# Cc19245/gaussian-splatting_CC-Comments

Hardware: AMD Instinct MI355X
Metric: train iters/sec (fwd+bwd rasterize) @1980x1080, 1M Gaussians (higher is better)
Workload: dtype f32; 1 GPU; C3: 1000000 Gaussians, SH deg 3, 1980x1080, mu=-5.0, seed 0; P=1000000, parallelism=single view

## Files before the change

__graft_entry__.py:

```python
import os
import subprocess
import sys

ROOT = os.path.dirname(os.path.abspath(__file__))
PKG = os.path.join(ROOT, "gaussian-splatting_cc-comments_amd")
CSRC = os.path.join(PKG, "csrc")
LIB = os.path.join(PKG, "libgsr_hip.so")
for p in (ROOT, PKG):
    if p not in sys.path:
        sys.path.insert(0, p)


def _stale(target, sources):
    if not os.path.exists(target):
        return True
    t = os.path.getmtime(target)
    return any(os.path.getmtime(s) > t for s in sources)


def build(force=False):
    srcs = [os.path.join(CSRC, f) for f in os.listdir(CSRC) if f.endswith((".hip", ".h", ".inc"))] + \
           [os.path.join(ROOT, "include", h) for h in ("gsr.h", "gsr_aux.h", "gsr_aa.h", "gsr_cam.h", "gsr_absgrad.h", "gsr_contrib.h", "gsr_features.h", "gsr_distortion.h", "gsr_median.h", "gsr_normals.h", "gsr_camera_model.h", "gsr_cam_cm.h")] + [os.path.join(CSRC, "Makefile")]
    if force or _stale(LIB, srcs):
        jobs = str(min(8, os.cpu_count() or 1))
        subprocess.check_call(["make", "-C", CSRC, "-j", jobs] + (["-B"] if force else []))
    subprocess.check_call(["make", "-C", os.path.join(ROOT, "tests", "cpp")], stdout=subprocess.DEVNULL)
    from oracle import oracle as _oracle
    _oracle.build(force=force)
    import diff_gaussian_rasterization
    from diff_gaussian_rasterization import _C
    _C.lib()


def smoke():
    import numpy as np
    import torch

    import gsr_scene
    from diff_gaussian_rasterization import GaussianRasterizationSettings, GaussianRasterizer
    from oracle import oracle

    assert torch.cuda.is_available(), "smoke() needs a GPU"
    dev = torch.device("cuda:0")
    scene = gsr_scene.make_scene(2000, -3.0, sh_degree=3, seed=3)
    cam = gsr_scene.make_camera(200, 120)
    to = lambda t: t.to(dev)
    means = to(scene.means3D).requires_grad_(True)
    shs = to(scene.shs).requires_grad_(True)
    opac = to(scene.opacities).requires_grad_(True)
    scales = to(scene.scales).requires_grad_(True)
    rots = to(scene.rotations).requires_grad_(True)
    means2D = torch.zeros_like(means, requires_grad=True)
    settings = GaussianRasterizationSettings(
        image_height=cam.image_height, image_width=cam.image_width, tanfovx=cam.tanfovx, tanfovy=cam.tanfovy,
        bg=to(scene.bg), scale_modifier=1.0, viewmatrix=to(cam.world_view_transform),
# ... 29 lines not shown
```

gaussian-splatting_cc-comments_amd/csrc/api.hip:

```cpp
#include <stdarg.h>
#include <stdio.h>
#include <string.h>

#include <atomic>
#include <cmath>
#include <mutex>
#include <string>
#include <vector>

#include "gsr_internal.h"
#include "../../include/gsr_aa.h"
#include "../../include/gsr_contrib.h"
#include "../../include/gsr_features.h"
#include "../../include/gsr_distortion.h"
#include "../../include/gsr_median.h"
#include "../../include/gsr_normals.h"

#define GSR_MAX_DEVICES 64
#ifndef GSR_COLOR_BESIDE_WGS
#define GSR_COLOR_BESIDE_WGS 2
#endif
#define GSR_COLOR_BESIDE_MAX_P 1500000

static thread_local char g_err[512] = "";

int gsr_fail(int code, const char* fmt, ...)
{
	va_list ap;
	va_start(ap, fmt);
	vsnprintf(g_err, sizeof g_err, fmt, ap);
	va_end(ap);
	return code;
}

int gsr_check_hip(hipError_t e, const char* what)
{
	if (e == hipSuccess) return GSR_OK;
	return gsr_fail(GSR_ERR_HIP, "%s: %s", what, hipGetErrorString(e));
}

int gsr_stage_done(hipStream_t s, int debug, const char* stage)
{
	hipError_t e = hipGetLastError();
	if (e != hipSuccess) return gsr_fail(GSR_ERR_HIP, "launch of %s failed: %s", stage, hipGetErrorString(e));
	if (debug & GSR_DEBUG_SYNC) {
		e = hipStreamSynchronize(s);
		if (e != hipSuccess) return gsr_fail(GSR_ERR_HIP, "[HIP ERROR] in stage %s: %s", stage, hipGetErrorString(e));
	}
	return GSR_OK;
}

extern "C" const char* gsr_last_error(void) { return g_err; }
extern "C" const char* gsr_version(void) { return "gsr-hip gfx950 r4"; }

struct ProfEntry { const char* name; hipEvent_t a, b; };
struct ProfRecorder {
	hipStream_t stream;
	bool on = false, open = false;
	std::vector<ProfEntry> ev;
	size_t used = 0;
	char only[64] = "";
};
static std::mutex g_prof_mu;
static std::vector<ProfRecorder*> g_prof;
static std::atomic<int> g_prof_active{0};

static ProfRecorder* prof_find(hipStream_t s, bool create)
{
	for (ProfRecorder* r : g_prof)
		if (r->stream == s) return r;
	if (!create) return nullptr;
	ProfRecorder* r = new ProfRecorder();
	r->stream = s;
	g_prof.push_back(r);
	return r;
}

static ProfEntry& prof_next(ProfRecorder* r, const char* name)
{
	if (r->used == r->ev.size()) {
		ProfEntry e;
		e.name = name;
		(void)hipEventCreate(&e.a);
		(void)hipEventCreate(&e.b);
		r->ev.push_back(e);
	}
// ... 266 lines not shown
{
	gsr_binning_layout l;
	gsr_binning_layout_of(P, R, W, H, &l);
	char* b = (char*)blob;
	GsrBinning bn;
	bn.point_list = (uint32_t*)(b + l.point_list);
	bn.point_list_alt = (uint32_t*)(b + l.point_list_alt);
	bn.tile_keys = (uint32_t*)(b + l.tile_keys);
	bn.tile_keys_alt = (uint32_t*)(b + l.tile_keys_alt);
	bn.sort_table = (void*)(b + l.sort_table);
	bn.checkpoints = (float4*)(b + l.checkpoints);
	return bn;
}

extern "C" uint32_t gsr_get_higher_msb(uint32_t n)
{
	uint32_t msb = sizeof(n) * 4;
	uint32_t step = msb;
	while (step > 1) {
		step /= 2;
		if (n >> msb) msb += step; else msb -= step;
	}
	if (n >> msb) msb++;
	return msb;
}

struct GsrThreadDevice {
	hipStream_t aux_stream = nullptr;
	hipEvent_t aux_fork = nullptr, aux_join = nullptr;
	uint32_t* status_host = nullptr;
	hipEvent_t status_event = nullptr;
	hipStream_t copy_stream = nullptr;
	hipEvent_t copy_fork = nullptr;
};
struct GsrThreadState { GsrThreadDevice dev[GSR_MAX_DEVICES]; };
static thread_local GsrThreadState g_thread;

extern "C" int gsr_thread_release(void)
{
	g_err[0] = 0;
	int rc = GSR_OK;
	for (int d = 0; d < GSR_MAX_DEVICES; d++) {
		GsrThreadDevice& t = g_thread.dev[d];
		if (t.aux_stream) { (void)hipStreamSynchronize(t.aux_stream); if (hipStreamDestroy(t.aux_stream) != hipSuccess) rc = GSR_ERR_HIP; }
		if (t.aux_fork && hipEventDestroy(t.aux_fork) != hipSuccess) rc = GSR_ERR_HIP;
		if (t.aux_join && hipEventDestroy(t.aux_join) != hipSuccess) rc = GSR_ERR_HIP;
		if (t.status_event && hipEventDestroy(t.status_event) != hipSuccess) rc = GSR_ERR_HIP;
		if (t.copy_stream) { (void)hipStreamSynchronize(t.copy_stream); if (hipStreamDestroy(t.copy_stream) != hipSuccess) rc = GSR_ERR_HIP; }
		if (t.copy_fork && hipEventDestroy(t.copy_fork) != hipSuccess) rc = GSR_ERR_HIP;
		if (t.status_host && hipHostFree(t.status_host) != hipSuccess) rc = GSR_ERR_HIP;
		t = GsrThreadDevice();
	}
	if (rc) { (void)hipGetLastError(); return gsr_fail(rc, "gsr_thread_release: a HIP resource could not be freed"); }
	return GSR_OK;
}

static bool gsr_helper_stream(hipStream_t* stream, hipEvent_t* e0, hipEvent_t* e1)
{
	if (*stream) return true;
	hipStream_t st = nullptr;
	hipEvent_t a = nullptr, b = nullptr;
	if (hipStreamCreateWithFlags(&st, hipStreamNonBlocking) == hipSuccess && hipEventCreateWithFlags(&a, hipEventDisableTiming) == hipSuccess &&
	    (!e1 || hipEventCreateWithFlags(&b, hipEventDisableTiming) == hipSuccess)) {
		*stream = st; *e0 = a;
		if (e1) *e1 = b;
		return true;
// ... 40 lines not shown
{
	g_err[0] = 0;
	hipStream_t s = (hipStream_t)stream;
	GsrPreprocessArgs a = in;
	const int P = a.P, width = a.W, height = a.H;
	if (!num_rendered_host) return gsr_fail(GSR_ERR_INVALID_ARGUMENT, "num_rendered_host is NULL");
	*num_rendered_host = 0;
	if (P < 0 || width <= 0 || height <= 0) return gsr_fail(GSR_ERR_INVALID_ARGUMENT, "bad P / image size");
	if (P == 0) return GSR_OK;
	if (!a.means3D || !a.opacities || !a.viewmatrix || (!a.projmatrix && !cm) || !geometry)
		return gsr_fail(GSR_ERR_INVALID_ARGUMENT, "gsr_forward_preprocess: required pointer is NULL");
	if (!a.colors_precomp && !a.shs)
		return gsr_fail(GSR_ERR_INVALID_ARGUMENT, "For non-RGB, provide precomputed Gaussian colors!");
	if (!a.colors_precomp && (a.M <= 0 || (a.D + 1) * (a.D + 1) > a.M || a.D < 0 || a.D > 3 || !a.cam_pos))
		return gsr_fail(GSR_ERR_INVALID_ARGUMENT, "SH degree %d needs %d coefficients, M = %d", a.D, (a.D + 1) * (a.D + 1), a.M);
	if (!a.cov3D_precomp && (!a.scales || !a.rotations))
		return gsr_fail(GSR_ERR_INVALID_ARGUMENT, "provide scales+rotations or cov3D_precomp");
	if (width > 65535 * GSR_TILE_X || height > 65535 * GSR_TILE_Y)
		return gsr_fail(GSR_ERR_INVALID_ARGUMENT, "image too large for 16-bit tile coordinates");
	if (!aligned16(geometry)) return gsr_fail(GSR_ERR_INVALID_ARGUMENT, "geometry buffer must be 16-byte aligned");

	if (a.leaf && (a.M > 1 && !a.shs_rest)) return gsr_fail(GSR_ERR_INVALID_ARGUMENT, "leaf mode: features_rest is NULL");
	if (a.leaf && a.M > 16) return gsr_fail(GSR_ERR_INVALID_ARGUMENT, "leaf mode: at most 16 SH coefficients (degree 3), M = %d", a.M);
	a.focal_y = height / (2.0f * a.tan_fovy);
	a.focal_x = width / (2.0f * a.tan_fovx);
	if (cm) { a.focal_x = cm->fx; a.focal_y = cm->fy; }
	a.g = gsr_geometry_view(geometry, P);

	int rc;
	int device = 0;
	if ((rc = gsr_check_hip(hipGetDevice(&device), "hipGetDevice"))) return rc;
	if (device < 0 || device >= GSR_MAX_DEVICES) return gsr_fail(GSR_ERR_INVALID_ARGUMENT, "device index %d not supported", device);
	GsrThreadDevice& td = g_thread.dev[device];
	const bool col_pairs = gsr_tilebin_applies(width, height) && !(debug & GSR_DEBUG_TILE_SORT);
	a.trim = (col_pairs && !(debug & GSR_DEBUG_NO_TRIM)) ? 1 : 0;
	const bool color = gsr_preprocess_needs_color(a);
#ifdef GSR_AB_FORCE_RADIX_DEPTH
	const bool bucket = false;
#else
	const bool bucket = gsr_bucket_sort_applies(P) && !(debug & GSR_DEBUG_RADIX_DEPTH);
#endif
	const bool beside = color && !(debug & (GSR_DEBUG_SYNC | GSR_DEBUG_SERIAL)) && !gsr_prof_records_all(s) &&
	                    gsr_helper_stream(&td.aux_stream, &td.aux_fork, &td.aux_join);
	GsrJoinOnExit join(s);
	gsr_launch_zero_status(a.g.status, s, beside ? td.aux_fork : nullptr);
	if (beside) {
		if ((rc = gsr_check_hip(hipStreamWaitEvent(td.aux_stream, td.aux_fork, 0), "hipStreamWaitEvent(fork)"))) return rc;
		gsr_launch_preprocess_color(a, td.aux_stream, P <= GSR_COLOR_BESIDE_MAX_P ? GSR_COLOR_BESIDE_WGS : 0, aux);
		if (hipEventRecord(td.aux_join, td.aux_stream) != hipSuccess) {
			(void)hipStreamSynchronize(td.aux_stream);
			return gsr_fail(GSR_ERR_HIP, "hipEventRecord(join) failed");
		}
		join.arm(td.aux_join);
	}
	const bool copy_beside = !(debug & (GSR_DEBUG_SYNC | GSR_DEBUG_SERIAL)) && !gsr_prof_records_all(s) &&
	                         gsr_helper_stream(&td.copy_stream, &td.copy_fork, nullptr);
	{
		GsrProfScope p(s, "preprocess");
		gsr_launch_preprocess(a, s, copy_beside ? td.copy_fork : nullptr, aux, aa, cm);
	}
	if ((rc = gsr_stage_done(s, debug, "preprocess"))) return rc;
	if (color && !beside) {
		GsrProfScope p(s, "preprocess_color");
		gsr_launch_preprocess_color(a, s, 0, aux);
	}
	if ((rc = gsr_stage_done(s, debug, "preprocess_color"))) return rc;

	if (!td.status_host) {
		if ((rc = gsr_check_hip(hipHostMalloc((void**)&td.status_host, GSR_STATUS_WORDS * 4, hipHostMallocDefault), "hipHostMalloc"))) return rc;
	}
	if (!td.status_event) {
		if ((rc = gsr_check_hip(hipEventCreateWithFlags(&td.status_event, hipEventDisableTiming), "hipEventCreate"))) return rc;
	}
	uint32_t* status_host = td.status_host;
	hipEvent_t ev = td.status_event;
	if (copy_beside && (rc = gsr_check_hip(hipStreamWaitEvent(td.copy_stream, td.copy_fork, 0), "hipStreamWaitEvent(copy fork)"))) return rc;
	hipStream_t cs = copy_beside ? td.copy_stream : s;
	GsrDrainOnExit drain;
	if (copy_beside) drain.arm(td.copy_stream);
	if ((rc = gsr_check_hip(hipMemcpyAsync(status_host, a.g.status, GSR_STATUS_WORDS * 4, hipMemcpyDeviceToHost, cs), "hipMemcpyAsync(num_rendered)"))) return rc;
	if ((rc = gsr_check_hip(hipEventRecord(ev, cs), "hipEventRecord"))) return rc;
	const uint32_t* bias = a.g.status + GSR_STATUS_NEGMIN;
	{
		GsrProfScope p(s, "depth_sort");
		if (bucket) {
			gsr_launch_depth_bucket_sort(a.g, P, col_pairs ? gsr_tilebin_seg(a.g, P) : nullptr, s);
			if (col_pairs) gsr_launch_tilebin_col_hist(a.g, P, 0, s, true);
			else gsr_launch_sorted_block_sums(a.g, P, 0, s);
		} else {
			gsr_radix_sort_passes(a.g.depth_keys, a.g.perm, a.g.depth_keys_alt, a.g.perm_alt, (size_t)P, 32, 4, 0, 3, a.g.sort_table, bias, 4, s);
			if (col_pairs) gsr_launch_tilebin_col_hist(a.g, P, 1, s);
			else gsr_launch_sorted_block_sums(a.g, P, 1, s);
			gsr_launch_slot_base_finish(a.g.slot_base, a.g.block_tiles, a.g.status, (size_t)P, s);
		}
	}
	if ((rc = gsr_stage_done(s, debug, "depth_sort"))) return rc;
	if ((rc = gsr_check_hip(hipEventSynchronize(ev), "hipEventSynchronize(num_rendered)"))) return rc;
// ... 981 lines not shown
```

gaussian-splatting_cc-comments_amd/csrc/gsr_internal.h:

```cpp
#pragma once
#include <hip/hip_runtime.h>
#include <hip/hip_ext.h>
#include <stddef.h>
#include <stdint.h>

#include <type_traits>

#include "../../include/gsr.h"
#include "../../include/gsr_aux.h"
#include "../../include/gsr_cam.h"
#include "../../include/gsr_absgrad.h"
#include "../../include/gsr_camera_model.h"
#include "../../include/gsr_cam_cm.h"
#include "gsr_device.h"

#define GSR_PREPROCESS_BLOCK 256
#define GSR_COUNT_PARTS 64
#define GSR_STATUS_NEGMIN (4 + GSR_COUNT_PARTS)
#define GSR_STATUS_MAX (4 + 2 * GSR_COUNT_PARTS)
#define GSR_STATUS_WORDS (4 + 3 * GSR_COUNT_PARTS)

#ifndef GSR_SLOT_COOP
#define GSR_SLOT_COOP 30
#endif
// ... 95 lines not shown
		if (aux == GSR_AUX_INVDEPTH) with_leaf(std::integral_constant<int, GSR_AUX_INVDEPTH>{}, AA);
		else if (aux) with_leaf(std::integral_constant<int, GSR_AUX_DEPTH>{}, AA);
		else with_leaf(std::integral_constant<int, 0>{}, AA);
	};
	if (aa) with_aux(std::true_type{});
	else with_aux(std::false_type{});
}

struct GsrPreprocessArgs {
	int P, D, M, W, H;
	const float* means3D;
	const float* shs;
	const float* colors_precomp;
	const float* opacities;
	const float* scales;
	float scale_modifier;
	const float* rotations;
	const float* cov3D_precomp;
	const float* viewmatrix;
	const float* projmatrix;
	const float* cam_pos;
	float tan_fovx, tan_fovy, focal_x, focal_y;
	int prefiltered;
	int trim;
	int* radii;
	GsrGeometry g;
	int leaf;
	const float* shs_rest;
};

void gsr_launch_preprocess(const GsrPreprocessArgs& a, hipStream_t s, hipEvent_t done, int aux, int aa, const gsr_camera_model* cm = nullptr);
void gsr_launch_zero_status(uint32_t* status, hipStream_t s, hipEvent_t done);
bool gsr_preprocess_needs_color(const GsrPreprocessArgs& a);
void gsr_launch_preprocess_color(const GsrPreprocessArgs& a, hipStream_t s, int wgs_per_cu, int aux);
void gsr_launch_mark_visible(int P, const float* means3D, const float* viewmatrix, uint8_t* present, hipStream_t s);

void gsr_launch_sorted_block_sums(GsrGeometry g, int P, int result_in_alt, hipStream_t s);
void gsr_launch_duplicate_keys(GsrGeometry g, int P, int W, void* keys, int key_bytes, uint32_t* vals, uint32_t* clear, size_t clear_words, hipStream_t s);
void gsr_launch_tile_ranges(const void* tile_keys, int key_bytes, int64_t R, uint2* ranges, int ntiles, uint32_t* valid, hipStream_t s);
void gsr_launch_tile_order(GsrImage img, int ntiles, bool backward, int64_t num_rendered, bool split, hipStream_t s, bool normalise_empty = false);
uint32_t gsr_tile_order_max_split(int ntiles);
uint32_t gsr_tile_order_max_segments(int ntiles);

bool gsr_tilebin_applies(int W, int H);
size_t gsr_tilebin_col_clear_words(size_t P);
size_t gsr_tilebin_col_table_bytes(size_t P);
size_t gsr_tilebin_row_clear_words(size_t R);
size_t gsr_tilebin_row_table_bytes(size_t R);
void gsr_launch_tilebin_col_hist(GsrGeometry g, int P, int result_in_alt, hipStream_t s, bool seg_ready = false);
uint4* gsr_tilebin_seg(GsrGeometry g, int P);
uint4* gsr_tilebin_recs(GsrGeometry g, int P);
void gsr_launch_tilebin_col_scatter(GsrGeometry g, int P, GsrBinning b, int64_t R, hipStream_t s);
void gsr_launch_tilebin_row_hist(GsrGeometry g, int P, GsrBinning b, int64_t R, hipStream_t s);
void gsr_launch_tilebin_row_scatter(GsrGeometry g, int P, GsrBinning b, int64_t R, uint2* ranges, int W, int H, hipStream_t s);

int gsr_radix_num_passes(int nbits_total);
size_t gsr_radix_table_bytes(size_t n);
size_t gsr_radix_clear_words(size_t n);
void gsr_launch_slot_base_finish(uint32_t* slot_base, const uint32_t* block_tiles, uint32_t* status, size_t n, hipStream_t s);
void gsr_radix_sort_passes(void* k0, uint32_t* v0, void* k1, uint32_t* v1, size_t n, int nbits_total, int npass_total,
                           int pass_first, int pass_count, void* table_mem, const uint32_t* bias, int key_bytes, hipStream_t s);
void gsr_radix_sort_u32(void* k0, uint32_t* v0, void* k1, uint32_t* v1, size_t n, int nbits_total, void* table_mem,
                        int* result_in_first, int clear_table, int key_bytes, hipStream_t s);
void gsr_radix_top_pass(const uint32_t* k0, uint32_t* k1, const uint2* rec_in, uint4* rec_out, size_t n, void* table_mem, const uint32_t* bias, hipStream_t s,
                        uint32_t* slot_base, const uint32_t* block_tiles, uint32_t* status);
int gsr_radix_top_chunks(size_t n);
#ifndef GSR_BUCKET_SORT_MAX_P
// ... 110 lines not shown
```

gaussian-splatting_cc-comments_amd/csrc/preprocess.hip:

```cpp
#include "gsr_internal.h"
#include "gsr_rect_trim.h"
#include "gsr_aa.h"
#include "gsr_camera_model.h"

__device__ __forceinline__ float gsr_sh_channel(int deg, const float* sh, int ch, float x, float y, float z)
{
#define SH(k) sh[(k) * 3 + ch]
	float result = GSR_SH_C0 * SH(0);
	if (deg > 0) {
		result = result - GSR_SH_C1 * y * SH(1) + GSR_SH_C1 * z * SH(2) - GSR_SH_C1 * x * SH(3);
		if (deg > 1) {
			float xx = x * x, yy = y * y, zz = z * z;
			float xy = x * y, yz = y * z, xz = x * z;
			result = result + GSR_SH_C2[0] * xy * SH(4) + GSR_SH_C2[1] * yz * SH(5) +
			         GSR_SH_C2[2] * (2.0f * zz - xx - yy) * SH(6) + GSR_SH_C2[3] * xz * SH(7) +
			         GSR_SH_C2[4] * (xx - yy) * SH(8);
			if (deg > 2) {
				result = result + GSR_SH_C3[0] * y * (3.0f * xx - yy) * SH(9) + GSR_SH_C3[1] * xy * z * SH(10) +
				         GSR_SH_C3[2] * y * (4.0f * zz - xx - yy) * SH(11) +
				         GSR_SH_C3[3] * z * (2.0f * zz - 3.0f * xx - 3.0f * yy) * SH(12) +
				         GSR_SH_C3[4] * x * (4.0f * zz - xx - yy) * SH(13) + GSR_SH_C3[5] * z * (xx - yy) * SH(14) +
				         GSR_SH_C3[6] * x * (xx - 3.0f * yy) * SH(15);
			}
		}
	}
#undef SH
	return result + 0.5f;
}

template <bool LEAF, int AUX, bool AA, bool CM>
__global__ void __launch_bounds__(GSR_PREPROCESS_BLOCK) gsr_preprocess_kernel(
	typename std::conditional<CM, GsrWithCameraModel<GsrPreprocessArgs>, GsrPreprocessArgs>::type a, uint32_t* __restrict__ clear, size_t clear_words,
	uint32_t* __restrict__ clear2, size_t clear2_words)
{
	const int idx = blockIdx.x * GSR_PREPROCESS_BLOCK + threadIdx.x;
	GsrVec3 p_orig = {0.f, 0.f, 0.f};
// ... 104 lines not shown
	for (int off = 32; off > 0; off >>= 1) {
		kneg = max(kneg, (uint32_t)__shfl_xor(kneg, off, 64));
		kmax = max(kmax, (uint32_t)__shfl_xor(kmax, off, 64));
	}
	if ((threadIdx.x & 63) == 63) { wsum[threadIdx.x >> 6] = incl; wneg[threadIdx.x >> 6] = kneg; wmax[threadIdx.x >> 6] = kmax; }
	__syncthreads();
	{
		uint32_t before = 0, t = 0;
#pragma unroll
		for (int w = 0; w < GSR_PREPROCESS_BLOCK / 64; w++) {
			if (w < (int)(threadIdx.x >> 6)) before += wsum[w];
			t += wsum[w];
		}
		if (idx < a.P) a.g.slot_base[idx] = before + incl - tiles;
		if (threadIdx.x == 0) {
			a.g.block_tiles[blockIdx.x] = t;
			uint32_t n2 = 0, m2 = 0;
#pragma unroll
			for (int w = 0; w < GSR_PREPROCESS_BLOCK / 64; w++) { n2 = max(n2, wneg[w]); m2 = max(m2, wmax[w]); }
			if (t) {
				const int part = blockIdx.x & (GSR_COUNT_PARTS - 1);
				atomicAdd(&a.g.status[4 + part], t);
				atomicMax(&a.g.status[GSR_STATUS_NEGMIN + part], n2);
				atomicMax(&a.g.status[GSR_STATUS_MAX + part], m2);
			}
		}
	}
	for (size_t w = (size_t)blockIdx.x * GSR_PREPROCESS_BLOCK + threadIdx.x; w < clear_words; w += (size_t)gridDim.x * GSR_PREPROCESS_BLOCK)
		clear[w] = 0u;
	for (size_t w = (size_t)blockIdx.x * GSR_PREPROCESS_BLOCK + threadIdx.x; w < clear2_words; w += (size_t)gridDim.x * GSR_PREPROCESS_BLOCK)
		clear2[w] = 0u;
}

template <bool LEAF, int AUX>
__global__ void __launch_bounds__(GSR_PREPROCESS_BLOCK) gsr_preprocess_color_kernel(GsrPreprocessArgs a, int sh_via_lds)
{
	__shared__ float4 s_sh[GSR_PREPROCESS_BLOCK / 64][32 * GSR_SH_ROW4];
	const int idx = blockIdx.x * GSR_PREPROCESS_BLOCK + threadIdx.x;
	GsrVec3 p_orig = {0.f, 0.f, 0.f};
	if (idx < a.P) { p_orig.x = a.means3D[3 * idx]; p_orig.y = a.means3D[3 * idx + 1]; p_orig.z = a.means3D[3 * idx + 2]; }
	float row[48];
	if (sh_via_lds) {
		const int lane = threadIdx.x & 63, wave = threadIdx.x >> 6;
		const int wave_first = blockIdx.x * GSR_PREPROCESS_BLOCK + wave * 64;
		const int nrows = min(64, a.P - wave_first);
		if (LEAF) {
			GsrShLinFetch v;
			gsr_sh_lin_fetch(v, a.shs, a.shs_rest, wave_first, max(nrows, 0), lane);
			float* lin = reinterpret_cast<float*>(s_sh[wave]);
#pragma unroll
			for (int half = 0; half < 2; half++) {
				gsr_sh_lin_commit_half(lin, v, lane, half);
				__builtin_amdgcn_wave_barrier();
				if ((lane >> 5) == half) gsr_sh_linh_row_get(lin, lane & 31, row);
				__builtin_amdgcn_wave_barrier();
			}
		} else {
			float4 v[12];
			gsr_sh_rows_fetch(v, a.shs, wave_first, max(nrows, 0), lane);
#pragma unroll
			for (int half = 0; half < 2; half++) {
				gsr_sh_rows_commit_half(s_sh[wave], v, nrows, lane, half);
				__builtin_amdgcn_wave_barrier();
				if ((lane >> 5) == half) gsr_sh_row_get(s_sh[wave], lane & 31, row);
				__builtin_amdgcn_wave_barrier();
			}
		}
	}
	if (idx >= a.P) return;
	if (gsr_transform_point_4x3(p_orig, a.viewmatrix).z <= 0.2f) return;

	float dx = p_orig.x - a.cam_pos[0], dy = p_orig.y - a.cam_pos[1], dz = p_orig.z - a.cam_pos[2];
	float len = sqrtf(dx * dx + dy * dy + dz * dz);
	dx = dx / len; dy = dy / len; dz = dz / len;
	const float* sh = a.shs + (size_t)idx * a.M * 3;
	float raw[3], ddir9[9];
	if (sh_via_lds) {
#pragma unroll
		for (int ch = 0; ch < 3; ch++) raw[ch] = gsr_sh_channel(a.D, row, ch, dx, dy, dz);
		gsr_sh_ddir9(a.D, row, dx, dy, dz, ddir9);
	} else {
		float sh_local[48];
		if (LEAF) {
			const int used = (a.D + 1) * (a.D + 1);
#pragma unroll
			for (int k = 0; k < 16; k++)
				if (k < used) {
#pragma unroll
					for (int ch = 0; ch < 3; ch++)
						sh_local[k * 3 + ch] = k == 0 ? a.shs[3 * (size_t)idx + ch] : a.shs_rest[((size_t)idx * (a.M - 1) + (k - 1)) * 3 + ch];
				}
			sh = sh_local;
		}
#pragma unroll
		for (int ch = 0; ch < 3; ch++) raw[ch] = gsr_sh_channel(a.D, sh, ch, dx, dy, dz);
		gsr_sh_ddir9(a.D, sh, dx, dy, dz, ddir9);
	}
#pragma unroll
	for (int k = 0; k < 9; k++) a.g.sh_ddir[(size_t)k * a.P + idx] = ddir9[k];
	uint8_t clamp_bits = 0;
	float rgb[3];
#pragma unroll
	for (int ch = 0; ch < 3; ch++) {
		const float v = raw[ch];
		if (v < 0) clamp_bits |= (uint8_t)(1u << ch);
		rgb[ch] = fmaxf(v, 0.0f);
	}
	a.g.clamped[idx] = clamp_bits;
	reinterpret_cast<float4*>(a.g.splat + idx)[2] =
		make_float4(rgb[0], rgb[1], rgb[2], AUX ? gsr_aux_value<AUX>(gsr_transform_point_4x3(p_orig, a.viewmatrix).z) : 0.f);
}

__global__ void gsr_zero_status_kernel(uint32_t* __restrict__ status)
{
	if (threadIdx.x < GSR_STATUS_WORDS) status[threadIdx.x] = 0u;
}
void gsr_launch_zero_status(uint32_t* status, hipStream_t s, hipEvent_t done)
{
	static_assert(GSR_STATUS_WORDS <= 256, "one workgroup zeroes the status words");
	gsr_launch(gsr_zero_status_kernel, dim3(1), dim3(256), 0, s, nullptr, done, status);
}

void gsr_launch_preprocess(const GsrPreprocessArgs& a, hipStream_t s, hipEvent_t done, int aux, int aa, const gsr_camera_model* cm)
{
	const int nb = (a.P + GSR_PREPROCESS_BLOCK - 1) / GSR_PREPROCESS_BLOCK;
	uint32_t* clear = (uint32_t*)a.g.sort_table;
	const size_t clear_words = gsr_radix_clear_words((size_t)a.P);
	uint32_t* clear2 = (uint32_t*)a.g.col_table;
	const size_t clear2_words = gsr_tilebin_col_clear_words((size_t)a.P);
	gsr_variant(a.leaf, aux, aa, [&](auto LEAF, auto AUX, auto AA) {
		if (cm) {
			GsrWithCameraModel<GsrPreprocessArgs> c;
			static_cast<GsrPreprocessArgs&>(c) = a;
			c.cm_model = cm->model; c.cm_cx = cm->cx; c.cm_cy = cm->cy;
			gsr_launch(gsr_preprocess_kernel<LEAF(), AUX(), AA(), true>, dim3(nb), dim3(GSR_PREPROCESS_BLOCK), 0, s, nullptr, done,
			           c, clear, clear_words, clear2, clear2_words);
			return;
		}
		gsr_launch(gsr_preprocess_kernel<LEAF(), AUX(), AA(), false>, dim3(nb), dim3(GSR_PREPROCESS_BLOCK), 0, s, nullptr, done,
		           a, clear, clear_words, clear2, clear2_words);
	});
}

bool gsr_preprocess_needs_color(const GsrPreprocessArgs& a) { return a.shs && !a.colors_precomp; }

void gsr_launch_preprocess_color(const GsrPreprocessArgs& a, hipStream_t s, int wgs_per_cu, int aux)
{
	const int nb = (a.P + GSR_PREPROCESS_BLOCK - 1) / GSR_PREPROCESS_BLOCK;
	const int sh_via_lds = (a.M == 16 && ((uintptr_t)a.shs & 15u) == 0 && !(a.leaf && ((uintptr_t)a.shs_rest & 15u) != 0)) ? 1 : 0;
	const size_t own = (size_t)(GSR_PREPROCESS_BLOCK / 64) * 32 * GSR_SH_ROW4 * sizeof(float4);
	const size_t share = wgs_per_cu > 0 ? (size_t)160 * 1024 / (size_t)wgs_per_cu : 0;
	const size_t throttle = share > own + 1024 ? share - own - 1024 : 0;
	gsr_variant(a.leaf, aux, false, [&](auto LEAF, auto AUX, auto) {
		gsr_launch(gsr_preprocess_color_kernel<LEAF(), AUX()>, dim3(nb), dim3(GSR_PREPROCESS_BLOCK), throttle, s, nullptr, nullptr, a, sh_via_lds);
	});
}

__global__ void gsr_mark_visible_kernel(int P, const float* means3D, const float* viewmatrix, uint8_t* present)
{
	const int idx = blockIdx.x * blockDim.x + threadIdx.x;
	if (idx >= P) return;
	GsrVec3 p = {means3D[3 * idx], means3D[3 * idx + 1], means3D[3 * idx + 2]};
	GsrVec3 pv = gsr_transform_point_4x3(p, viewmatrix);
	present[idx] = !(pv.z <= 0.2f);
}

void gsr_launch_mark_visible(int P, const float* means3D, const float* viewmatrix, uint8_t* present, hipStream_t s)
{
	hipLaunchKernelGGL(gsr_mark_visible_kernel, dim3((P + 255) / 256), dim3(256), 0, s, P, means3D, viewmatrix, present);
}
```

gaussian-splatting_cc-comments_amd/diff_gaussian_rasterization/_C.py:

```python
import ctypes
import math
import os
from typing import NamedTuple

import torch

_HERE = os.path.dirname(os.path.abspath(__file__))
_LIB_PATH = os.path.join(os.path.dirname(_HERE), "libgsr_hip.so")
_lib = None

_vp = ctypes.c_void_p
_i = ctypes.c_int
_i64 = ctypes.c_int64
_f = ctypes.c_float
_sz = ctypes.c_size_t


class GeometryLayout(ctypes.Structure):
    _fields_ = [(n, _sz) for n in ("splat", "depth_keys", "depth_keys_alt", "perm", "perm_alt", "tiles_touched", "rect",
                                   "slot_base", "clamped", "sh_ddir", "status", "scan_temp", "sort_table", "col_table", "rshape", "total")]


class ImageLayout(ctypes.Structure):
    _fields_ = [(n, _sz) for n in ("final_C", "final_T", "n_contrib", "ranges", "tile_max_contrib", "tile_order", "total")]
# ... 77 lines not shown


def use_library(path):
    global _LIB_PATH
    if _lib is not None:
        raise RuntimeError("use_library() must be called before the library is first loaded")
    _LIB_PATH = os.path.abspath(path)


def lib():
    global _lib
    if _lib is not None:
        return _lib
    if not os.path.exists(_LIB_PATH):
        raise RuntimeError(
            f"{_LIB_PATH} not found: build it with `python -c 'import __graft_entry__ as g; g.build()'` "
            "(hipcc --offload-arch=gfx950).  There is no CPU fallback for the rasterizer.")
    L = ctypes.CDLL(_LIB_PATH)
    L.gsr_last_error.restype = ctypes.c_char_p
    L.gsr_version.restype = ctypes.c_char_p
    L.gsr_geometry_bytes.restype = _sz
    L.gsr_geometry_bytes.argtypes = [_i]
    L.gsr_image_bytes.restype = _sz
    L.gsr_image_bytes.argtypes = [_i, _i]
    L.gsr_binning_bytes.restype = _sz
    L.gsr_binning_bytes.argtypes = [_i, _i64, _i, _i]
    L.gsr_backward_scratch_bytes.restype = _sz
    L.gsr_backward_scratch_bytes.argtypes = [_i, _i64]
    L.gsr_geometry_layout_of.argtypes = [_i, ctypes.POINTER(GeometryLayout)]
    L.gsr_image_layout_of.argtypes = [_i, _i, ctypes.POINTER(ImageLayout)]
    L.gsr_binning_layout_of.argtypes = [_i, _i64, _i, _i, ctypes.POINTER(BinningLayout)]
    L.gsr_get_higher_msb.restype = ctypes.c_uint32
    L.gsr_get_higher_msb.argtypes = [ctypes.c_uint32]
    L.gsr_forward_preprocess.restype = _i
    L.gsr_forward_preprocess.argtypes = [_i, _i, _i, _i, _i, _vp, _vp, _vp, _vp, _vp, _f, _vp, _vp, _vp, _vp, _vp,
                                         _f, _f, _i, _vp, _vp, ctypes.POINTER(_i64), _vp, _i]
    L.gsr_forward_render.restype = _i
    L.gsr_forward_render.argtypes = [_i, _i64, _i, _i, _vp, _vp, _vp, _vp, _vp, _vp, _vp, _i]
    L.gsr_backward.restype = _i
    L.gsr_backward.argtypes = [_i, _i, _i, _i64, _i, _i] + [_vp] * 5 + [_f] + [_vp] * 5 + [_f, _f] + [_vp] * 16 + [_i]
    L.gsr_mark_visible.restype = _i
    L.gsr_mark_visible.argtypes = [_i, _vp, _vp, _vp, _vp, _vp]
    L.gsr_sh_grad_from_views.restype = _i
    L.gsr_sh_grad_from_views.argtypes = [_i, _i, _i, _i, _vp, _vp, _vp, _i64, _vp, _vp]
    L.gsr_backward_blend.restype = _i
    L.gsr_backward_blend.argtypes = [ctypes.POINTER(BackwardArgs)]
    L.gsr_backward_gaussians.restype = _i
    L.gsr_backward_gaussians.argtypes = [ctypes.POINTER(BackwardArgs), _i, _i, _i]
    L.gsr_thread_release.restype = _i
    L.gsr_thread_release.argtypes = []
    L.gsr_profile_begin.restype = _i
    L.gsr_profile_begin.argtypes = [_vp]
    L.gsr_profile_begin_only.restype = _i
    L.gsr_profile_begin_only.argtypes = [_vp, ctypes.c_char_p]
    L.gsr_profile_end.restype = _i
    L.gsr_profile_end.argtypes = [_vp, ctypes.POINTER(KernelTime), _i]
    leaf_pre = [_i] * 5 + [_vp] * 5 + [_f] + [_vp] * 4 + [_f, _f, _i, _vp, _vp, ctypes.POINTER(_i64), _vp, _i]
    L.gsr_forward_preprocess_leaf.restype = _i
    L.gsr_forward_preprocess_leaf.argtypes = leaf_pre
    L.gsr_adam_step.restype = _i
    L.gsr_adam_step.argtypes = [_i, _vp, ctypes.c_double, ctypes.c_double, ctypes.c_double, _vp, _vp]
    pa, pb = ctypes.POINTER(AuxArgs), ctypes.POINTER(BackwardArgs)
    L.gsr_aux_bytes.restype = _sz
    L.gsr_aux_bytes.argtypes = [_i64, _i, _i]
    L.gsr_aux_layout_of.restype = _i
    L.gsr_aux_layout_of.argtypes = [_i64, _i, _i, ctypes.POINTER(AuxLayout)]
# ... 785 lines not shown
        elif out.shape != (P, M, 3) or out.dtype != torch.float32 or out.device != dev or not out.is_contiguous():
            raise RuntimeError("sh_grad_from_views: out must be a contiguous float32 (P,M,3) tensor on the device of means3D")
        _check(L.gsr_sh_grad_from_views(P, int(degree), int(M), V, _ptr(means3D), _ptr(cam_pos), _ptr(dL_dRGB), view_stride,
                                        _ptr(out), _stream(dev)))
    return out


def mark_visible(means3D, viewmatrix, projmatrix):
    if not means3D.is_cuda:
        raise RuntimeError("means3D must be a HIP (cuda) tensor; the HIP rasterizer has no CPU path")
    L = lib()
    dev = means3D.device
    P = int(means3D.size(0))
    present = torch.zeros((P,), dtype=torch.bool, device=dev)
    if P != 0:
        means3D = _dev_f32(means3D, dev, "means3D")
        viewmatrix = _dev_f32(viewmatrix, dev, "viewmatrix")
        projmatrix = _dev_f32(projmatrix, dev, "projmatrix")
        with torch.cuda.device(dev):
            _check(L.gsr_mark_visible(P, _ptr(means3D), _ptr(viewmatrix), _ptr(projmatrix), _ptr(present), _stream(dev)))
    return present


def thread_release():
    _check(lib().gsr_thread_release())


def geometry_layout(P):
    o = GeometryLayout()
    _check(lib().gsr_geometry_layout_of(P, ctypes.byref(o)))
    return o


def image_layout(W, H):
    o = ImageLayout()
    _check(lib().gsr_image_layout_of(W, H, ctypes.byref(o)))
    return o


def binning_layout(P, R, W, H):
    o = BinningLayout()
    _check(lib().gsr_binning_layout_of(P, R, W, H, ctypes.byref(o)))
    return o


def profile_begin(only=None, device=None):
    stream = _stream(torch.device("cuda", torch.cuda.current_device()) if device is None else device)
    _check(lib().gsr_profile_begin_only(stream, None if only is None else only.encode()))


def profile_end(capacity=256, device=None):
    stream = _stream(torch.device("cuda", torch.cuda.current_device()) if device is None else device)
    arr = (KernelTime * capacity)()
    n = lib().gsr_profile_end(stream, arr, capacity)
    return [(arr[k].name.decode(), float(arr[k].ms)) for k in range(n)]


def aux_layout(R, W, H):
    lay = AuxLayout()
    _check(lib().gsr_aux_layout_of(int(R), int(W), int(H), ctypes.byref(lay)))
    return {n: getattr(lay, n) for n, _ in AuxLayout._fields_}
```

Measured before the change: 1000 it/s.

## Bound side-stream color preprocess with a persistent grid instead of LDS throttling

The SH color preprocess kernel becomes a grid-stride loop whose grid is capped at wgs_per_cu times the CU count when it runs beside the main preprocess. This replaces the old trick of padding dynamic LDS to limit residency. It also adds launch_bounds occupancy 4, an optional quarter-size LDS staging path, and nondeterministic-value initialisation to reduce register and spill pressure. The intent is to limit how much the overlapped color kernel competes with the main preprocess while lowering launch and occupancy waste. The cost is fewer workgroups in flight for the color work.

```diff
diff --git a/__graft_entry__.py b/__graft_entry__.py
--- a/__graft_entry__.py
+++ b/__graft_entry__.py
@@ -20,7 +20,7 @@
 
 def build(force=False):
     srcs = [os.path.join(CSRC, f) for f in os.listdir(CSRC) if f.endswith((".hip", ".h", ".inc"))] + \
-           [os.path.join(ROOT, "include", h) for h in ("gsr.h", "gsr_aux.h", "gsr_aa.h", "gsr_cam.h", "gsr_absgrad.h", "gsr_contrib.h", "gsr_features.h", "gsr_distortion.h", "gsr_median.h", "gsr_normals.h", "gsr_camera_model.h", "gsr_cam_cm.h")] + [os.path.join(CSRC, "Makefile")]
+           [os.path.join(ROOT, "include", h) for h in ("gsr.h", "gsr_aux.h", "gsr_aa.h", "gsr_cam.h", "gsr_absgrad.h", "gsr_contrib.h", "gsr_features.h", "gsr_distortion.h", "gsr_median.h", "gsr_normals.h", "gsr_camera_model.h", "gsr_cam_cm.h", "gsr_color_launch.h")] + [os.path.join(CSRC, "Makefile")]
     if force or _stale(LIB, srcs):
         jobs = str(min(8, os.cpu_count() or 1))
         subprocess.check_call(["make", "-C", CSRC, "-j", jobs] + (["-B"] if force else []))
diff --git a/gaussian-splatting_cc-comments_amd/csrc/api.hip b/gaussian-splatting_cc-comments_amd/csrc/api.hip
--- a/gaussian-splatting_cc-comments_amd/csrc/api.hip
+++ b/gaussian-splatting_cc-comments_amd/csrc/api.hip
@@ -15,6 +15,7 @@
 #include "../../include/gsr_distortion.h"
 #include "../../include/gsr_median.h"
 #include "../../include/gsr_normals.h"
+#include "../../include/gsr_color_launch.h"
 
 #define GSR_MAX_DEVICES 64
 #ifndef GSR_COLOR_BESIDE_WGS
@@ -52,6 +53,7 @@
 
 extern "C" const char* gsr_last_error(void) { return g_err; }
 extern "C" const char* gsr_version(void) { return "gsr-hip gfx950 r4"; }
+extern "C" int gsr_color_beside_wgs(void) { return GSR_COLOR_BESIDE_WGS; }
 
 struct ProfEntry { const char* name; hipEvent_t a, b; };
 struct ProfRecorder {
@@ -384,6 +386,7 @@
 	hipEvent_t status_event = nullptr;
 	hipStream_t copy_stream = nullptr;
 	hipEvent_t copy_fork = nullptr;
+	int cu_count = 0;
 };
 struct GsrThreadState { GsrThreadDevice dev[GSR_MAX_DEVICES]; };
 static thread_local GsrThreadState g_thread;
@@ -490,6 +493,7 @@
 	if ((rc = gsr_check_hip(hipGetDevice(&device), "hipGetDevice"))) return rc;
 	if (device < 0 || device >= GSR_MAX_DEVICES) return gsr_fail(GSR_ERR_INVALID_ARGUMENT, "device index %d not supported", device);
 	GsrThreadDevice& td = g_thread.dev[device];
+	if (td.cu_count <= 0 && (rc = gsr_check_hip(hipDeviceGetAttribute(&td.cu_count, hipDeviceAttributeMultiprocessorCount, device), "hipDeviceGetAttribute(CU count)"))) return rc;
 	const bool col_pairs = gsr_tilebin_applies(width, height) && !(debug & GSR_DEBUG_TILE_SORT);
 	a.trim = (col_pairs && !(debug & GSR_DEBUG_NO_TRIM)) ? 1 : 0;
 	const bool color = gsr_preprocess_needs_color(a);
@@ -504,7 +508,7 @@
 	gsr_launch_zero_status(a.g.status, s, beside ? td.aux_fork : nullptr);
 	if (beside) {
 		if ((rc = gsr_check_hip(hipStreamWaitEvent(td.aux_stream, td.aux_fork, 0), "hipStreamWaitEvent(fork)"))) return rc;
-		gsr_launch_preprocess_color(a, td.aux_stream, P <= GSR_COLOR_BESIDE_MAX_P ? GSR_COLOR_BESIDE_WGS : 0, aux);
+		gsr_launch_preprocess_color(a, td.aux_stream, P <= GSR_COLOR_BESIDE_MAX_P ? GSR_COLOR_BESIDE_WGS : 0, td.cu_count, aux);
 		if (hipEventRecord(td.aux_join, td.aux_stream) != hipSuccess) {
 			(void)hipStreamSynchronize(td.aux_stream);
 			return gsr_fail(GSR_ERR_HIP, "hipEventRecord(join) failed");
@@ -520,7 +524,7 @@
 	if ((rc = gsr_stage_done(s, debug, "preprocess"))) return rc;
 	if (color && !beside) {
 		GsrProfScope p(s, "preprocess_color");
-		gsr_launch_preprocess_color(a, s, 0, aux);
+		gsr_launch_preprocess_color(a, s, 0, td.cu_count, aux);
 	}
 	if ((rc = gsr_stage_done(s, debug, "preprocess_color"))) return rc;
 
diff --git a/gaussian-splatting_cc-comments_amd/csrc/gsr_internal.h b/gaussian-splatting_cc-comments_amd/csrc/gsr_internal.h
--- a/gaussian-splatting_cc-comments_amd/csrc/gsr_internal.h
+++ b/gaussian-splatting_cc-comments_amd/csrc/gsr_internal.h
@@ -151,7 +151,7 @@
 void gsr_launch_preprocess(const GsrPreprocessArgs& a, hipStream_t s, hipEvent_t done, int aux, int aa, const gsr_camera_model* cm = nullptr);
 void gsr_launch_zero_status(uint32_t* status, hipStream_t s, hipEvent_t done);
 bool gsr_preprocess_needs_color(const GsrPreprocessArgs& a);
-void gsr_launch_preprocess_color(const GsrPreprocessArgs& a, hipStream_t s, int wgs_per_cu, int aux);
+void gsr_launch_preprocess_color(const GsrPreprocessArgs& a, hipStream_t s, int wgs_per_cu, int cu_count, int aux);
 void gsr_launch_mark_visible(int P, const float* means3D, const float* viewmatrix, uint8_t* present, hipStream_t s);
 
 void gsr_launch_sorted_block_sums(GsrGeometry g, int P, int result_in_alt, hipStream_t s);
diff --git a/gaussian-splatting_cc-comments_amd/csrc/preprocess.hip b/gaussian-splatting_cc-comments_amd/csrc/preprocess.hip
--- a/gaussian-splatting_cc-comments_amd/csrc/preprocess.hip
+++ b/gaussian-splatting_cc-comments_amd/csrc/preprocess.hip
@@ -2,6 +2,7 @@
 #include "gsr_rect_trim.h"
 #include "gsr_aa.h"
 #include "gsr_camera_model.h"
+#include "../../include/gsr_color_launch.h"
 
 __device__ __forceinline__ float gsr_sh_channel(int deg, const float* sh, int ch, float x, float y, float z)
 {
@@ -172,83 +173,131 @@
 		clear2[w] = 0u;
 }
 
+#ifndef GSR_COLOR_STAGE_ROWS
+#define GSR_COLOR_STAGE_ROWS 32
+#endif
+#if GSR_COLOR_STAGE_ROWS == 32
+#define GSR_COLOR_ROWS_COMMIT gsr_sh_rows_commit_half
+#define GSR_COLOR_LIN_COMMIT gsr_sh_lin_commit_half
+#define GSR_COLOR_LIN_GET gsr_sh_linh_row_get
+#else
+__device__ __forceinline__ void gsr_sh_rows_commit_quarter(float4* __restrict__ rows, const float4* __restrict__ v, int nrows, int lane, int q)
+{
+	const int e = lane & 3, r0 = gsr_sh_rowmap_store(lane >> 2);
+#pragma unroll
+	for (int it = 0; it < 3; it++)
+		if (16 * q + r0 < nrows) rows[r0 * GSR_SH_ROW4 + 4 * it + e] = v[3 * q + it];
+}
+__device__ __forceinline__ void gsr_sh_lin_commit_quarter(float* __restrict__ lin, const GsrShLinFetch& v, int lane, int q)
+{
+#pragma unroll
+	for (int i = 0; i < 3; i++) {
+		const int e = lane + 64 * i;
+		if (e / 48 == q) lin[16 * 45 + e - 48 * q] = v.dc[i];
+	}
+#pragma unroll
+	for (int it = 0; it < 12; it++) {
+		const int f = it * 64 + lane;
+		if (f / 180 == q) *reinterpret_cast<float4*>(lin + 4 * (f - 180 * q)) = v.r[it];
+	}
+}
+__device__ __forceinline__ void gsr_sh_linq_row_get(const float* __restrict__ lin, int l, float* __restrict__ row48)
+{
+#pragma unroll
+	for (int c = 0; c < 3; c++) row48[c] = lin[16 * 45 + 3 * l + c];
+#pragma unroll
+	for (int j = 0; j < 45; j++) row48[3 + j] = lin[45 * l + j];
+}
+#define GSR_COLOR_ROWS_COMMIT gsr_sh_rows_commit_quarter
+#define GSR_COLOR_LIN_COMMIT gsr_sh_lin_commit_quarter
+#define GSR_COLOR_LIN_GET gsr_sh_linq_row_get
+#endif
 template <bool LEAF, int AUX>
-__global__ void __launch_bounds__(GSR_PREPROCESS_BLOCK) gsr_preprocess_color_kernel(GsrPreprocessArgs a, int sh_via_lds)
-{
-	__shared__ float4 s_sh[GSR_PREPROCESS_BLOCK / 64][32 * GSR_SH_ROW4];
-	const int idx = blockIdx.x * GSR_PREPROCESS_BLOCK + threadIdx.x;
-	GsrVec3 p_orig = {0.f, 0.f, 0.f};
-	if (idx < a.P) { p_orig.x = a.means3D[3 * idx]; p_orig.y = a.means3D[3 * idx + 1]; p_orig.z = a.means3D[3 * idx + 2]; }
-	float row[48];
-	if (sh_via_lds) {
-		const int lane = threadIdx.x & 63, wave = threadIdx.x >> 6;
-		const int wave_first = blockIdx.x * GSR_PREPROCESS_BLOCK + wave * 64;
-		const int nrows = min(64, a.P - wave_first);
-		if (LEAF) {
-			GsrShLinFetch v;
-			gsr_sh_lin_fetch(v, a.shs, a.shs_rest, wave_first, max(nrows, 0), lane);
-			float* lin = reinterpret_cast<float*>(s_sh[wave]);
-#pragma unroll
-			for (int half = 0; half < 2; half++) {
-				gsr_sh_lin_commit_half(lin, v, lane, half);
-				__builtin_amdgcn_wave_barrier();
-				if ((lane >> 5) == half) gsr_sh_linh_row_get(lin, lane & 31, row);
-				__builtin_amdgcn_wave_barrier();
-			}
-		} else {
-			float4 v[12];
-			gsr_sh_rows_fetch(v, a.shs, wave_first, max(nrows, 0), lane);
-#pragma unroll
-			for (int half = 0; half < 2; half++) {
-				gsr_sh_rows_commit_half(s_sh[wave], v, nrows, lane, half);
-				__builtin_amdgcn_wave_barrier();
-				if ((lane >> 5) == half) gsr_sh_row_get(s_sh[wave], lane & 31, row);
-				__builtin_amdgcn_wave_barrier();
-			}
-		}
-	}
-	if (idx >= a.P) return;
-	if (gsr_transform_point_4x3(p_orig, a.viewmatrix).z <= 0.2f) return;
-
-	float dx = p_orig.x - a.cam_pos[0], dy = p_orig.y - a.cam_pos[1], dz = p_orig.z - a.cam_pos[2];
-	float len = sqrtf(dx * dx + dy * dy + dz * dz);
-	dx = dx / len; dy = dy / len; dz = dz / len;
-	const float* sh = a.shs + (size_t)idx * a.M * 3;
-	float raw[3], ddir9[9];
-	if (sh_via_lds) {
-#pragma unroll
-		for (int ch = 0; ch < 3; ch++) raw[ch] = gsr_sh_channel(a.D, row, ch, dx, dy, dz);
-		gsr_sh_ddir9(a.D, row, dx, dy, dz, ddir9);
-	} else {
-		float sh_local[48];
-		if (LEAF) {
-			const int used = (a.D + 1) * (a.D + 1);
-#pragma unroll
-			for (int k = 0; k < 16; k++)
-				if (k < used) {
-#pragma unroll
-					for (int ch = 0; ch < 3; ch++)
-						sh_local[k * 3 + ch] = k == 0 ? a.shs[3 * (size_t)idx + ch] : a.shs_rest[((size_t)idx * (a.M - 1) + (k - 1)) * 3 + ch];
+__global__ void __launch_bounds__(GSR_PREPROCESS_BLOCK, 4) gsr_preprocess_color_kernel(GsrPreprocessArgs a, int sh_via_lds)
+{
+	__shared__ float4 s_sh[GSR_PREPROCESS_BLOCK / 64][GSR_COLOR_STAGE_ROWS * GSR_SH_ROW4];
+	const int nb = (a.P + GSR_PREPROCESS_BLOCK - 1) / GSR_PREPROCESS_BLOCK;
+#pragma unroll 1
+	for (int b = blockIdx.x; b < nb; b += gridDim.x) {
+		const int idx = b * GSR_PREPROCESS_BLOCK + threadIdx.x;
+		GsrVec3 p_orig = {0.f, 0.f, 0.f};
+		if (idx < a.P) { p_orig.x = a.means3D[3 * idx]; p_orig.y = a.means3D[3 * idx + 1]; p_orig.z = a.means3D[3 * idx + 2]; }
+		float row[48];
+#pragma unroll
+		for (int k = 0; k < 48; k++) row[k] = __builtin_nondeterministic_value(row[k]);
+		if (sh_via_lds) {
+			int lane = threadIdx.x & 63;
+			const int wave = threadIdx.x >> 6;
+			asm volatile("" : "+v"(lane));
+			const int wave_first = b * GSR_PREPROCESS_BLOCK + wave * 64;
+			const int nrows = min(64, a.P - wave_first);
+			if (LEAF) {
+				GsrShLinFetch v;
+				gsr_sh_lin_fetch(v, a.shs, a.shs_rest, wave_first, max(nrows, 0), lane);
+				float* lin = reinterpret_cast<float*>(s_sh[wave]);
+#pragma unroll
+				for (int half = 0; half < 64 / GSR_COLOR_STAGE_ROWS; half++) {
+					GSR_COLOR_LIN_COMMIT(lin, v, lane, half);
+					__builtin_amdgcn_wave_barrier();
+					if ((unsigned)lane / GSR_COLOR_STAGE_ROWS == (unsigned)half) GSR_COLOR_LIN_GET(lin, (unsigned)lane % GSR_COLOR_STAGE_ROWS, row);
+					__builtin_amdgcn_wave_barrier();
 				}
-			sh = sh_local;
-		}
-#pragma unroll
-		for (int ch = 0; ch < 3; ch++) raw[ch] = gsr_sh_channel(a.D, sh, ch, dx, dy, dz);
-		gsr_sh_ddir9(a.D, sh, dx, dy, dz, ddir9);
-	}
-#pragma unroll
-	for (int k = 0; k < 9; k++) a.g.sh_ddir[(size_t)k * a.P + idx] = ddir9[k];
-	uint8_t clamp_bits = 0;
-	float rgb[3];
-#pragma unroll
-	for (int ch = 0; ch < 3; ch++) {
-		const float v = raw[ch];
-		if (v < 0) clamp_bits |= (uint8_t)(1u << ch);
-		rgb[ch] = fmaxf(v, 0.0f);
-	}
-	a.g.clamped[idx] = clamp_bits;
-	reinterpret_cast<float4*>(a.g.splat + idx)[2] =
-		make_float4(rgb[0], rgb[1], rgb[2], AUX ? gsr_aux_value<AUX>(gsr_transform_point_4x3(p_orig, a.viewmatrix).z) : 0.f);
+			} else {
+				float4 v[12];
+				gsr_sh_rows_fetch(v, a.shs, wave_first, max(nrows, 0), lane);
+#pragma unroll
+				for (int half = 0; half < 64 / GSR_COLOR_STAGE_ROWS; half++) {
+					GSR_COLOR_ROWS_COMMIT(s_sh[wave], v, nrows, lane, half);
+					__builtin_amdgcn_wave_barrier();
+					if ((unsigned)lane / GSR_COLOR_STAGE_ROWS == (unsigned)half) gsr_sh_row_get(s_sh[wave], (unsigned)lane % GSR_COLOR_STAGE_ROWS, row);
+					__builtin_amdgcn_wave_barrier();
+				}
+			}
+		}
+		if (idx < a.P && !(gsr_transform_point_4x3(p_orig, a.viewmatrix).z <= 0.2f)) {
+			float dx = p_orig.x - a.cam_pos[0], dy = p_orig.y - a.cam_pos[1], dz = p_orig.z - a.cam_pos[2];
+			float len = sqrtf(dx * dx + dy * dy + dz * dz);
+			dx = dx / len; dy = dy / len; dz = dz / len;
+			const float* sh = a.shs + (size_t)idx * a.M * 3;
+			float raw[3], ddir9[9];
+			if (sh_via_lds) {
+#pragma unroll
+				for (int ch = 0; ch < 3; ch++) raw[ch] = gsr_sh_channel(a.D, row, ch, dx, dy, dz);
+				gsr_sh_ddir9(a.D, row, dx, dy, dz, ddir9);
+			} else {
+				float sh_local[48];
+#pragma unroll
+				for (int k = 0; k < 48; k++) sh_local[k] = __builtin_nondeterministic_value(sh_local[k]);
+				if (LEAF) {
+					const int used = (a.D + 1) * (a.D + 1);
+#pragma unroll
+					for (int k = 0; k < 16; k++)
+						if (k < used) {
+#pragma unroll
+							for (int ch = 0; ch < 3; ch++)
+								sh_local[k * 3 + ch] = k == 0 ? a.shs[3 * (size_t)idx + ch] : a.shs_rest[((size_t)idx * (a.M - 1) + (k - 1)) * 3 + ch];
+						}
+					sh = sh_local;
+				}
+#pragma unroll
+				for (int ch = 0; ch < 3; ch++) raw[ch] = gsr_sh_channel(a.D, sh, ch, dx, dy, dz);
+				gsr_sh_ddir9(a.D, sh, dx, dy, dz, ddir9);
+			}
+#pragma unroll
+			for (int k = 0; k < 9; k++) a.g.sh_ddir[(size_t)k * a.P + idx] = ddir9[k];
+			uint8_t clamp_bits = 0;
+			float rgb[3];
+#pragma unroll
+			for (int ch = 0; ch < 3; ch++) {
+				const float v = raw[ch];
+				if (v < 0) clamp_bits |= (uint8_t)(1u << ch);
+				rgb[ch] = fmaxf(v, 0.0f);
+			}
+			a.g.clamped[idx] = clamp_bits;
+			reinterpret_cast<float4*>(a.g.splat + idx)[2] =
+				make_float4(rgb[0], rgb[1], rgb[2], AUX ? gsr_aux_value<AUX>(gsr_transform_point_4x3(p_orig, a.viewmatrix).z) : 0.f);
+		}
+	}
 }
 
 __global__ void gsr_zero_status_kernel(uint32_t* __restrict__ status)
@@ -284,15 +333,22 @@
 
 bool gsr_preprocess_needs_color(const GsrPreprocessArgs& a) { return a.shs && !a.colors_precomp; }
 
-void gsr_launch_preprocess_color(const GsrPreprocessArgs& a, hipStream_t s, int wgs_per_cu, int aux)
-{
-	const int nb = (a.P + GSR_PREPROCESS_BLOCK - 1) / GSR_PREPROCESS_BLOCK;
+extern "C" void gsr_color_launch_shape(int P, int cu_count, int wgs_per_cu, int* grid, size_t* dynamic_lds_bytes)
+{
+	const int64_t nb = ((int64_t)(P > 0 ? P : 0) + GSR_PREPROCESS_BLOCK - 1) / GSR_PREPROCESS_BLOCK;
+	const int64_t limit = (wgs_per_cu > 0 && cu_count > 0) ? (int64_t)wgs_per_cu * cu_count : nb;
+	if (grid) *grid = (int)(nb < limit ? nb : limit);
+	if (dynamic_lds_bytes) *dynamic_lds_bytes = 0;
+}
+
+void gsr_launch_preprocess_color(const GsrPreprocessArgs& a, hipStream_t s, int wgs_per_cu, int cu_count, int aux)
+{
+	int grid = 0;
+	size_t dynamic_lds = 0;
+	gsr_color_launch_shape(a.P, cu_count, wgs_per_cu, &grid, &dynamic_lds);
 	const int sh_via_lds = (a.M == 16 && ((uintptr_t)a.shs & 15u) == 0 && !(a.leaf && ((uintptr_t)a.shs_rest & 15u) != 0)) ? 1 : 0;
-	const size_t own = (size_t)(GSR_PREPROCESS_BLOCK / 64) * 32 * GSR_SH_ROW4 * sizeof(float4);
-	const size_t share = wgs_per_cu > 0 ? (size_t)160 * 1024 / (size_t)wgs_per_cu : 0;
-	const size_t throttle = share > own + 1024 ? share - own - 1024 : 0;
 	gsr_variant(a.leaf, aux, false, [&](auto LEAF, auto AUX, auto) {
-		gsr_launch(gsr_preprocess_color_kernel<LEAF(), AUX()>, dim3(nb), dim3(GSR_PREPROCESS_BLOCK), throttle, s, nullptr, nullptr, a, sh_via_lds);
+		gsr_launch(gsr_preprocess_color_kernel<LEAF(), AUX()>, dim3(grid), dim3(GSR_PREPROCESS_BLOCK), dynamic_lds, s, nullptr, nullptr, a, sh_via_lds);
 	});
 }
 
diff --git a/gaussian-splatting_cc-comments_amd/diff_gaussian_rasterization/_C.py b/gaussian-splatting_cc-comments_amd/diff_gaussian_rasterization/_C.py
--- a/gaussian-splatting_cc-comments_amd/diff_gaussian_rasterization/_C.py
+++ b/gaussian-splatting_cc-comments_amd/diff_gaussian_rasterization/_C.py
@@ -133,6 +133,11 @@
     L.gsr_binning_layout_of.argtypes = [_i, _i64, _i, _i, ctypes.POINTER(BinningLayout)]
     L.gsr_get_higher_msb.restype = ctypes.c_uint32
     L.gsr_get_higher_msb.argtypes = [ctypes.c_uint32]
+    if hasattr(L, "gsr_color_launch_shape"):
+        L.gsr_color_launch_shape.restype = None
+        L.gsr_color_launch_shape.argtypes = [_i, _i, _i, ctypes.POINTER(_i), ctypes.POINTER(_sz)]
+        L.gsr_color_beside_wgs.restype = _i
+        L.gsr_color_beside_wgs.argtypes = []
     L.gsr_forward_preprocess.restype = _i
     L.gsr_forward_preprocess.argtypes = [_i, _i, _i, _i, _i, _vp, _vp, _vp, _vp, _vp, _f, _vp, _vp, _vp, _vp, _vp,
                                          _f, _f, _i, _vp, _vp, ctypes.POINTER(_i64), _vp, _i]
@@ -984,6 +989,16 @@
     return o
 
 
+def color_launch_shape(P, cu_count, wgs_per_cu):
+    grid, lds = _i(-1), _sz(1)
+    lib().gsr_color_launch_shape(int(P), int(cu_count), int(wgs_per_cu), ctypes.byref(grid), ctypes.byref(lds))
+    return int(grid.value), int(lds.value)
+
+
+def color_beside_wgs():
+    return int(lib().gsr_color_beside_wgs())
+
+
 def image_layout(W, H):
     o = ImageLayout()
     _check(lib().gsr_image_layout_of(W, H, ctypes.byref(o)))
diff --git a/include/gsr_color_launch.h b/include/gsr_color_launch.h
--- /dev/null
+++ b/include/gsr_color_launch.h
@@ -0,0 +1,12 @@
+#ifndef GSR_COLOR_LAUNCH_H_INCLUDED
+#define GSR_COLOR_LAUNCH_H_INCLUDED
+#include "gsr.h"
+#ifdef __cplusplus
+extern "C" {
+#endif
+void gsr_color_launch_shape(int P, int cu_count, int wgs_per_cu, int* grid, size_t* dynamic_lds_bytes);
+int gsr_color_beside_wgs(void);
+#ifdef __cplusplus
+}
+#endif
+#endif
```

Result: no change. 998.0 it/s (-0.3%).
